# griffithlab/regtools

Measured on AMD Instinct MI355X. Metric: alignments/sec + junctions/sec, junctions extract, 1/2/4/8 MI355X, higher is better.
Workload: dtype u8/u32 integer; 1 GPU; configs[1]: synthetic 50000000-read 101 bp BAM per GPU, ~15% reads with one N-op, junctions extract -s XS; reads_per_gpu=50000000, seed=1, bgzf_members=169426, compressed_bytes_per_gpu=533101619, inflated_bytes_per_gpu=11060000978

## Files before the change

regtools_amd/csrc/api_internal.h:

```cpp
#pragma once
#include "../../include/regtools_amd.h"

#include <hip/hip_runtime.h>
#include <stdarg.h>
#include <stdio.h>
#include <stdlib.h>
#include <string.h>

#include <algorithm>
#include <atomic>
#include <condition_variable>
#include <charconv>
#include <chrono>
#include <map>
#include <memory>
#include <mutex>
#include <string>
#include <thread>
#include <unordered_map>
#include <vector>

#include "cse_host.h"
#include "host_io.h"
#include "worker_pool.h"
// ... 320 lines not shown
    CallIndex(const uint8_t *index, size_t index_len) : bai(index), bai_len(index_len), th([this] {
        ok = bai && normalize_index(bai, bai_len, image, bai, bai_len) && parse_bai(bai, bai_len, bi, false); }) {}
    void join() { if (th.joinable()) th.join(); }
    ~CallIndex() { join(); }
};

struct MemberDiscovery {
    rgx_ctx *c = nullptr; hipStream_t st = nullptr;
    const uint8_t *d_bam = nullptr; size_t bam_len = 0;
    const uint32_t *d_true_sizes = nullptr;
    Scalars *d_sc = nullptr, *h_sc = nullptr;
    uint32_t n_cand = 0;
    uint64_t *cand = nullptr;
    uint32_t *nx[2] = {nullptr, nullptr}, *c_isize = nullptr, *c_reach = nullptr, *c_rank = nullptr, *c_isz2 = nullptr, *c_tmp = nullptr;
    Member *d_members = nullptr;
    StageGuard g_cand, g_members;
    int candidates(bool guarded, char *err, size_t errlen) {
        DevBuf &b_disc = c->buf(Buf::discover), &b_cand = c->buf(Buf::cand), &b_members = c->buf(Buf::members);
        const uint32_t n_tiles = (uint32_t)((bam_len + kMagicTile - 1) / kMagicTile);
        HIP_TRY(b_disc.ensure((size_t)n_tiles * 4 + scan_tmp_words(n_tiles) * 4 + 256));
        Carve wd(b_disc);
        uint32_t *tile_cnt = wd.u32(n_tiles), *tile_tmp = wd.u32(scan_tmp_words(n_tiles)); CARVE_TRY(wd, "discover");
        launch_magic_count(d_bam, bam_len, n_tiles, tile_cnt, st);
        launch_scan_u32(tile_cnt, tile_cnt, n_tiles, &d_sc->n_cand, tile_tmp, st);
        HIP_TRY(fetch_scalar(d_sc, h_sc, h_sc->n_cand, st));
        HIP_TRY(hipStreamSynchronize(st));
        n_cand = h_sc->n_cand;
        if (n_cand == 0) return kGoOn;
        const size_t N = n_cand, guard_bytes = guarded ? kGuardWords * 4 : 0;
        HIP_TRY(b_cand.ensure(N * 8 + N * 4 * 6 + scan_tmp_words(n_cand) * 4 + guard_bytes + 256));
        HIP_TRY(b_members.ensure((N + 1) * sizeof(Member) + guard_bytes));
        Carve wc(b_cand);
        cand = wc.u64(n_cand);
        uint32_t *guard_at = guarded ? wc.u32(kGuardWords) : nullptr;
        nx[0] = wc.u32(n_cand); nx[1] = wc.u32(n_cand);
        c_isize = wc.u32(n_cand); c_reach = wc.u32(n_cand); c_rank = wc.u32(n_cand); c_isz2 = wc.u32(n_cand); c_tmp = wc.u32(scan_tmp_words(n_cand));
        CARVE_TRY(wc, "cand");
        d_members = b_members.as<Member>();
        if (guarded) { g_cand.arm(guard_at, st); g_members.arm((uint32_t *)(d_members + N), st); }
        launch_magic_fill(d_bam, bam_len, n_tiles, tile_cnt, cand, st);
        return kGoOn;
    }
    void chain(uint64_t root2) {
        launch_member_link(d_bam, bam_len, cand, n_cand, nx[0], c_isize, c_reach, root2, st);
        int cur = 0;
        for (uint32_t span = 1; span < n_cand; span <<= 1) { launch_member_jump(n_cand, nx[cur], nx[cur ^ 1], c_reach, st); cur ^= 1; }
        launch_member_jump(n_cand, nx[cur], nx[cur ^ 1], c_reach, st);
        launch_scan_u32(c_reach, c_rank, n_cand, &d_sc->n_members, c_tmp, st);
// ... 82 lines not shown
        if (!split_B) return hipSuccess;
        split_B = false;
        return hipStreamWaitEvent(st, split_ev, 0);
    }
    bool spec = false; uint32_t mean_rec = 0;
    BamHeader hdr; int32_t n_ref = 0;
    uint64_t lim = 0, pos0 = 0; bool chain_ended = false;
    ExtractCfg cfg{}; SegGeom geom{}; uint32_t seg_bytes = 0;
    std::vector<SegChunk> seg_chunks;
    const uint8_t *arena = nullptr; uint64_t span = 0; uint32_t n_seg = 0, n_rec = 0; bool lite_walk = false;
    uint64_t *seg_start[2] = {nullptr, nullptr}, *seg_exit[2] = {nullptr, nullptr};
    uint32_t *seg_cnt[2] = {nullptr, nullptr}, *seg_base = nullptr;
    uint32_t *seg_iter_e = nullptr, *seg_long_e = nullptr, *seg_long_base_e = nullptr;
    uint16_t *seg_cp = nullptr;
    int cur = 0;
    int frame(uint32_t n_s, uint32_t walk_from, bool &ended) {
        DevBuf &b_tmp = c->buf(Buf::tmp);
        launch_seg_walk(arena, geom, n_s, n_ref, seg_start[cur], seg_exit[cur], seg_cnt[cur], seg_cp, st, walk_from);
        for (int iter = 0;; ++iter) {
            HIP_TRY(hipMemsetAsync(&d_sc->framing, 0xff, sizeof d_sc->framing, st));
            launch_seg_verify(arena, geom, n_s, seg_start[cur], seg_exit[cur], seg_cnt[cur], seg_start[cur ^ 1], seg_exit[cur ^ 1],
                              seg_cnt[cur ^ 1], &d_sc->framing.disagree, seg_cp, st);
            cur ^= 1;
            launch_scan_u32(seg_cnt[cur], seg_base, n_s, &d_sc->n_rec, b_tmp.as<uint32_t>(), st);
            HIP_TRY(fetch(h_sc->n_rec));
            HIP_TRY(fetch(h_sc->framing));
            if (spec && iter == 0) HIP_TRY(fetch_verdict());
            HIP_TRY(hipStreamSynchronize(st));
            if (spec && iter == 0 && !verdict_clean()) {
                mark("inflate verdict: not clean, starting over device-resident");
                if (gated) { c->gate_distrust = true; if (trace) fprintf(stderr,
                    "[rgx trace] arrival gate: verdict not clean, this context no longer uses it\n"); }
                return restart(Restart::verdict_not_clean);
            }
            ++P.framing_sweeps;
            const Scalars::Framing &fr = h_sc->framing;
            if (fr.chain_end != 0xffffffffu) ended = true;
            if (fr.chain_end != 0xffffffffu && (fr.chain_end < fr.disagree || (fr.disagree == 0xffffffffu && geom.chunks))) {
                launch_seg_truncate(geom, n_s, fr.chain_end, seg_start[cur], seg_exit[cur], seg_cnt[cur], st);
                launch_scan_u32(seg_cnt[cur], seg_base, n_s, &d_sc->n_rec, b_tmp.as<uint32_t>(), st);
                HIP_TRY(fetch(h_sc->n_rec));
                HIP_TRY(hipStreamSynchronize(st));
                break;
            }
            if (fr.disagree == 0xffffffffu) break;
            if (iter > 1 << 20) return fail(err, errlen, RGX_ERR_FORMAT, "regtools_amd: record framing did not converge\n");
        }
        return kGoOn;
    }
    uint32_t sA = 0;
    bool emit_parts_ok = false; uint32_t emit_parts = 0, emit_rows = 0; size_t ev_lay = 0;
    EventSoA ev_e{};
    static constexpr size_t kEventRowBytes = 8 * sizeof(uint32_t) + 1;
    EventSoA ev_layout(Carve &w, size_t E) {
        EventSoA v; memset(&v, 0, sizeof v);
        v.tid = w.u32(E); v.start = w.u32(E); v.ilen_cls = w.u32(E); v.ts = w.u32(E); v.te = w.u32(E);
        if (want_read_span) { v.rpos = w.u32(E); v.rend = w.u32(E); }
        if (p->barcodes) v.read = w.u32(E);
        v.strand = w.u8(E);
        return v;
    }
    size_t soa_cap = 0;
    ReadSoA soa{};
    uint32_t *ev_base = nullptr, *long_list = nullptr;
// ... 58 lines not shown
```

regtools_amd/csrc/api_records.cpp:

```cpp
#include "api_internal.h"

int EventsRun::stage_footers_and_header() {
    DevBuf &b_arena = c->buf(Buf::arena), &b_hdr = c->buf(Buf::hdr_arena), &b_lens = c->buf(Buf::inflate_scratch);
    BamHeader hdr_host;
    spec = overlap && !d_true_sizes && !geom_chunked_hint && host_bam_header(h_bam, std::min<size_t>(bam_len, (size_t)8 << 20), hdr_host, nullptr, &mean_rec);
    if (spec) h_sc->inflate = h_sc->inflate_early = InflateStatus{0xffffffffu, 0xffffffffu};
    else {
        HIP_TRY(join_B());
        HIP_TRY(fetch_verdict());
        HIP_TRY(hipStreamSynchronize(st));
    }
    if (!d_true_sizes) {
        auto size_trouble = [](const InflateStatus &s) { return s.first_bad != 0xffffffffu &&
            (s.code == 12u  || s.code == 10u ); };
        bool lies = size_trouble(h_sc->inflate) || size_trouble(h_sc->inflate_early);
        if (!lies && stop < n_members_all) {
            Member ms; uint8_t two[2] = {0, 0};
            HIP_TRY(member_at(stop, ms));
            if (ms.isize == 0 && ms.clen >= 2) {
                if (h_bam && ms.cpos + 2 <= bam_len) memcpy(two, h_bam + ms.cpos, 2);
                else { HIP_TRY(hipMemcpyAsync(two, d_bam + ms.cpos, 2, hipMemcpyDeviceToHost, st)); HIP_TRY(hipStreamSynchronize(st)); }
            }
            lies = !(ms.isize == 0 && two[0] == 3 && two[1] == 0) && ms.isize != 0xffffffffu;
        }
// ... 234 lines not shown
            if (reaches_J && trace) fprintf(stderr,
                "[rgx trace] early tail: a record of the prefix ends at %llu, behind the inflated part (%llu): one pass\n", (unsigned long long)exit_J,
                (unsigned long long)ep.upos);
            const bool slow_J = P.framing_sweeps - sweeps0 > 2;
            P.framing_sweeps = sweeps0;
            const uint64_t span_J = (uint64_t)sJ * seg_bytes;
            if (h_sc->wait_timed_out) { c->early_distrust = true; if (trace) fprintf(stderr,
                "[rgx trace] early tail: a wait for a part's waves timed out, this context no longer uses it\n"); }
            if (h_sc->wait_timed_out || ended_J || slow_J || reaches_J || !n_rec_J || span_J / n_rec_J > kSparseRecordBytes ||
                (sA && n_rec_J > soa_cap)) { early = false; sA = 0; emit_parts_ok = false; emit_parts = 0; emit_rows = 0; break; }
            if (!sA) {
                { const int rc = soa_layout((size_t)((double)n_rec_J * ((double)n_seg / sJ) * 1.125) + 65536); if (rc != kGoOn) return rc; }
                if (lite_walk) { cfg.insane_out = &d_sc->insane; HIP_TRY(hipMemsetAsync(&d_sc->insane, 0, 4, st)); h_sc->insane = 0; }
            }
            launch_decode_seg(arena, geom, sJ, seg_start[cur], seg_base, seg_cnt[cur], cfg, soa, seg_iter_e, seg_long_e, seg_cp, true, st, sA);
            if (!sA) {
                DevBuf &b_ev0 = c->buf(Buf::events);
                ev_lay = b_ev0.cap > 256 ? (b_ev0.cap - 256) / kEventRowBytes : 0;
                emit_parts_ok = ev_lay >= 4096;
                if (emit_parts_ok) { HIP_TRY(b_tmp.ensure(scan_tmp_words((uint32_t)std::min<size_t>(soa_cap, 0xffffffffu)) * 4 + 64));
                    Carve w(b_ev0); ev_e = ev_layout(w, ev_lay); CARVE_TRY(w, "events"); }
            }
            if (emit_parts_ok && emit_parts < kGateParts - 1) {
                launch_scan_u32(soa.n_ev + emit_rows, ev_base + emit_rows, n_rec_J - emit_rows, d_sc->part_events + emit_parts, b_tmp.as<uint32_t>(), st);
                launch_emit_short(arena, n_rec_J, cfg, soa, ev_base, ev_e, st, emit_rows, d_sc->part_events, emit_parts, (uint32_t)std::min<size_t>(ev_lay,
                    0xffffffffu));
                emit_rows = n_rec_J; ++emit_parts;
            }
            sA = sJ;
            mark("early tail: part framed and decoded");
        }
        HIP_TRY(join_B());
        const int rcF = frame(n_seg, sA, chain_ended);
        if (rcF != kGoOn) return rcF;
        n_rec = h_sc->n_rec;
    } else HIP_TRY(join_B());
    if (spec && !n_seg) {
        HIP_TRY(fetch_verdict());
        HIP_TRY(hipStreamSynchronize(st));
        if (!verdict_clean()) {
            mark("inflate verdict: not clean, nothing framed, starting over device-resident");
            return restart(Restart::verdict_not_clean_unframed);
        }
    }
    if (chain_ended) P.stream_ended = true;
    if (chain_ended && geom.chunks && m_hi < n_members_all && !path.to_file_end) {
        mark("region: chain ended, re-reading to the end of the file");
// ... 4 lines not shown

    return kGoOn;
}

int EventsRun::stage_decode() {
    DevBuf &b_tmp = c->buf(Buf::tmp);
    if (n_rec) {
        const size_t R = n_rec;
        const uint32_t s_from = sA && (R > soa_cap || chain_ended) ? 0 : sA;
        if (!s_from) { const int rc = soa_layout(R); if (rc != kGoOn) return rc; emit_parts_ok = false; }
        HIP_TRY(b_tmp.ensure(scan_tmp_words(n_rec) * 4 + 64));
        uint32_t *seg_iter = sA ? seg_iter_e : seg_cnt[cur ^ 1], *seg_long = sA ? seg_long_e : (uint32_t *)seg_start[cur ^ 1], *seg_long_base = sA ?
            seg_long_base_e : (uint32_t *)seg_exit[cur ^ 1];
        if (geom.chunks) {
            cfg.stop_out = &d_sc->stop_rule.index; cfg.stop_index = 0xffffffffu;
            HIP_TRY(hipMemsetAsync(&d_sc->stop_rule.index, 0xff, 4, st));
            HIP_TRY(hipMemsetAsync(&d_sc->stop_rule.last_pass, 0, 4, st));
        }
        if (!s_from && lite_walk) { cfg.insane_out = &d_sc->insane; HIP_TRY(hipMemsetAsync(&d_sc->insane, 0, 4, st)); h_sc->insane = 0; }
        for (int pass = 0; pass < 2; ++pass) {
            launch_decode_seg(arena, geom, n_seg, seg_start[cur], seg_base, seg_cnt[cur], cfg, soa, seg_iter, seg_long, seg_cp,
                              span / n_rec <= kSparseRecordBytes, st, s_from);
            if (emit_parts_ok && s_from) {
                launch_scan_u32(soa.n_ev + emit_rows, ev_base + emit_rows, n_rec - emit_rows, d_sc->part_events + emit_parts, b_tmp.as<uint32_t>(), st);
                launch_emit_short(arena, n_rec, cfg, soa, ev_base, ev_e, st, emit_rows, d_sc->part_events, emit_parts,
                    (uint32_t)std::min<size_t>(ev_lay, 0xffffffffu));
                HIP_TRY(fetch(h_sc->part_events));
            } else launch_scan_u32(soa.n_ev, ev_base, n_rec, &d_sc->counts.n_events, b_tmp.as<uint32_t>(), st);
            launch_scan_u32(seg_iter, seg_iter, n_seg, &d_sc->counts.n_iterated, b_tmp.as<uint32_t>(), st);
            launch_scan_u32(seg_long, seg_long_base, n_seg, &d_sc->counts.n_long, b_tmp.as<uint32_t>(), st);
            HIP_TRY(fetch(h_sc->counts));
            if (cfg.stop_out) HIP_TRY(fetch(h_sc->stop_rule));
            if (cfg.insane_out) HIP_TRY(fetch(h_sc->insane));
            if (cfg.abort_out) HIP_TRY(fetch(h_sc->abort_row));
            if (cfg.odd_count) HIP_TRY(fetch(h_sc->odd_aux));
            HIP_TRY(hipStreamSynchronize(st));
            if (cfg.insane_out && h_sc->insane) {
                mark("decode: a record fails bam_read1's test, starting over with the full walk");
                return restart(Restart::record_fails_full_test);
            }
            if (pass || !cfg.stop_out || h_sc->stop_rule.index == 0xffffffffu || h_sc->stop_rule.last_pass <= h_sc->stop_rule.index + 1) break;
            cfg.stop_index = h_sc->stop_rule.index;
        }
        if (cfg.abort_out && h_sc->abort_row != 0xffffffffu && h_sc->abort_row < (cfg.stop_out ? cfg.stop_index : 0xffffffffu))
            return fail(err, errlen, RGX_ERR_ABORT,
                "regtools_amd: record %u has an auxiliary field of unknown type in front of its strand or barcode tag: the reference abort()s here\n",
                h_sc->abort_row);
        n_events = h_sc->counts.n_events; n_long = h_sc->counts.n_long;
        if (emit_parts_ok && s_from) {
            uint64_t tot = 0;
            for (uint32_t k = 0; k <= emit_parts && k < kGateParts; ++k) tot += h_sc->part_events[k];
            if (tot > ev_lay || tot > 0xffffffffull || n_long) {
                emit_parts_ok = false;
                launch_scan_u32(soa.n_ev, ev_base, n_rec, &d_sc->counts.n_events, b_tmp.as<uint32_t>(), st);
                HIP_TRY(fetch(h_sc->counts.n_events));
                HIP_TRY(hipStreamSynchronize(st));
                n_events = h_sc->counts.n_events;
            } else n_events = (uint32_t)tot;
        }
        n_iterated = h_sc->counts.n_iterated;
        if (cfg.odd_count && h_sc->odd_aux) {
            const uint32_t cap = h_sc->odd_aux;
            DevBuf &b_odd = c->buf(Buf::odd_aux);
            HIP_TRY(b_odd.ensure((size_t)cap * 12 + 16));
            HIP_TRY(hipMemsetAsync(&d_sc->odd_aux, 0, 4, st));
            launch_collect_odd_aux(arena, soa, n_rec, cap, &d_sc->odd_aux, b_odd.as<int32_t>(), st);
            HIP_TRY(fetch(h_sc->odd_aux));
            HIP_TRY(hipStreamSynchronize(st));
            const uint32_t n_odd = std::min(h_sc->odd_aux, cap);
            std::vector<int32_t> rows((size_t)n_odd * 3);
            if (n_odd) { HIP_TRY(hipMemcpyAsync(rows.data(), b_odd.p, (size_t)n_odd * 12, hipMemcpyDeviceToHost, st)); HIP_TRY(hipStreamSynchronize(st)); }
            for (uint32_t k = 0; k < n_odd; ++k) P.odd_aux.push_back(Prep::OddAux{rows[3 * (size_t)k], rows[3 * (size_t)k + 1], rows[3 * (size_t)k + 2]});
        }
        if (geom.chunks && p->n_shards > 1 && h_sc->stop_rule.index != 0xffffffffu) P.stream_ended = true;
        if (n_long) launch_long_fill(n_seg, seg_base, seg_cnt[cur], seg_long_base, cfg, soa, long_list, st);
    }
    HIP_TRY(hipEventRecord(c->ev[4], st));
    mark("decode+count (sync)");
// ... 49 lines not shown
```

regtools_amd/csrc/api_reduce.cpp:

```cpp
#include "api_internal.h"

int reduce_events(rgx_ctx *c, EventSoA ev, uint32_t n_events, uint32_t group_bits, uint32_t ilen_bits, const uint32_t *rank_of_group_host,
                         uint32_t n_groups, HostRows &R, char *err, size_t errlen, bool view_only, RowMap *row_map, TableSink *sink, bool allow_preagg) {
    hipStream_t st = c->stream;
    Scalars *d_sc = c->buf(Buf::scalars).as<Scalars>(), *h_sc = (Scalars *)c->pinned;
    DevBuf &b_sort = c->buf(Buf::sort), &b_uni = c->buf(Buf::unique);
    c->last_rows_valid = false;
    uint32_t n_unique = 0;
    UniqueSoA u; memset(&u, 0, sizeof u);
    const uint32_t *final_perm = nullptr;
    uint32_t *chrom_rank_rows = nullptr;
    R = HostRows();
    if (n_events) {
        const bool preagg = !row_map && allow_preagg;
        PartialSoA pr; memset(&pr, 0, sizeof pr);
        uint32_t *ev_flag = nullptr, *ev_flag_tmp = nullptr;
        EventSoA sev = ev;
        uint32_t n_s = n_events;
        if (preagg) {
            DevBuf &b_par = c->buf(Buf::partials);
            const size_t Ev = n_events;
            HIP_TRY(b_par.ensure(Ev * 4 * 9 + scan_tmp_words(n_events) * 4 + 512));
            Carve q(b_par);
            pr.tid = q.u32(Ev); pr.start = q.u32(Ev); pr.ilen_cls = q.u32(Ev); pr.ts = q.u32(Ev); pr.te = q.u32(Ev);
            pr.count = q.u32(Ev); pr.first = q.u32(Ev); pr.last = q.u32(Ev); ev_flag = q.u32(Ev); ev_flag_tmp = q.u32(scan_tmp_words(n_events));
            CARVE_TRY(q, "partials");
            HIP_TRY(hipMemsetAsync(&d_sc->counts.n_partial, 0, 4, st));
            launch_preagg(ev, n_events, pr, &d_sc->counts.n_partial, st);
            HIP_TRY(fetch_scalar(d_sc, h_sc, h_sc->counts.n_partial, st));
            HIP_TRY(hipStreamSynchronize(st));
            n_s = h_sc->counts.n_partial;
            memset(&sev, 0, sizeof sev);
            sev.tid = pr.tid; sev.start = pr.start; sev.ilen_cls = pr.ilen_cls; sev.ts = pr.ts; sev.te = pr.te;
        }
        const size_t E = n_s;
        const size_t rtmp = radix_tmp_words(n_s) + scan_tmp_words(n_s) + 64;
        HIP_TRY(b_sort.ensure(E * 4 * 6 + rtmp * 4 + 256));
        Carve q(b_sort);
        uint32_t *perm0 = q.u32(E), *perm1 = q.u32(E), *key0 = q.u32(E), *key1 = q.u32(E);
        uint32_t *head = q.u32(E), *seg_excl = q.u32(E), *tmp = q.u32(rtmp); CARVE_TRY(q, "sort");
        RadixSort by_key{{perm0, perm1}, tmp, n_s, st, {key0, key1}};
        by_key.by_keyed(sev.ilen_cls, ilen_bits);
        by_key.by_keyed(sev.start, 32);
        by_key.by_keyed(sev.tid, group_bits);
        const uint32_t *sorted = by_key.sorted();
        launch_heads(sev, sorted, n_s, head, st);
        launch_scan_u32(head, seg_excl, n_s, &d_sc->counts.n_unique, tmp, st);
        HIP_TRY(fetch_scalar(d_sc, h_sc, h_sc->counts.n_unique, st));
        HIP_TRY(hipStreamSynchronize(st));
        n_unique = h_sc->counts.n_unique;

        const size_t U = n_unique;
        const size_t utmp = radix_tmp_words(n_unique) + 64;
        HIP_TRY(b_uni.ensure(U * 4 * 13 + U + utmp * 4 + 256));
        Carve w(b_uni);
        u.tid = w.u32(U); u.start = w.u32(U); u.end = w.u32(U); u.ts_min = w.u32(U); u.te_max = w.u32(U); u.count = w.u32(U);
        u.first_seen = w.u32(U); u.last_seen = w.u32(U); u.name_rank = w.u32(U);
        uint32_t *head_pos = w.u32(U); chrom_rank_rows = w.u32(U);
        uint32_t *uperm0 = w.u32(U), *uperm1 = w.u32(U), *utmp_p = w.u32(utmp);
        u.strand = w.u8(U); CARVE_TRY(w, "unique");
        launch_fill_u32(u.ts_min, 0xffffffffu, U, st);
        launch_fill_u32(u.te_max, 0u, U, st);
        if (preagg) {
            launch_fill_u32(u.count, 0u, U, st);
            launch_fill_u32(u.first_seen, 0xffffffffu, U, st);
            launch_fill_u32(u.last_seen, 0u, U, st);
            launch_reduce_partials(pr, sorted, head, seg_excl, n_s, u, st);
            HIP_TRY(hipMemsetAsync(ev_flag, 0, (size_t)n_events * 4, st));
            launch_reduce_finish_partials(ev.strand, n_unique, u, ev_flag, st);
            launch_scan_u32(ev_flag, ev_flag, n_events, nullptr, ev_flag_tmp, st);
            launch_name_rank(n_unique, ev_flag, u, st);
        } else {
            launch_reduce(ev, sorted, head, seg_excl, n_events, u, head_pos, st);
            if (row_map) {
                DevBuf &b_map = c->buf(Buf::row_map);
                HIP_TRY(b_map.ensure((E + U) * 4 + 256));
                Carve wm(b_map);
                row_map->ev_urow = wm.u32(E); row_map->urow_pos = wm.u32(U); CARVE_TRY(wm, "row_map");
                launch_event_urow(sorted, head, seg_excl, n_events, row_map->ev_urow, st);
            }
            uint32_t *first_flag = head;
            HIP_TRY(hipMemsetAsync(first_flag, 0, E * 4, st));
            launch_reduce_finish(ev, sorted, n_events, n_unique, head_pos, u, first_flag, st);
            launch_scan_u32(first_flag, seg_excl, n_events, nullptr, tmp, st);
            launch_name_rank(n_unique, seg_excl, u, st);
        }

        uint32_t rk = 0;
        for (uint32_t i = 0; i < n_groups; ++i) rk = std::max(rk, rank_of_group_host[i]);
// ... 71 lines not shown
    b.len = q.u32(E); b.h_lo = q.u32(E); b.h_hi = q.u32(E); b.row = q.u32(E);
    uint32_t *perm0 = q.u32(E), *perm1 = q.u32(E), *head = q.u32(E), *seg_excl = q.u32(E);
    uint32_t *pair_row = q.u32(E), *pair_first = q.u32(E), *pair_pos = q.u32(E), *pair_len = q.u32(E), *pair_count = q.u32(E);
    uint32_t *tmp = q.u32(rtmp); CARVE_TRY(q, "barcodes");
    uint32_t *flags = &d_sc->barcodes.not_string;
    HIP_TRY(hipMemsetAsync(flags, 0, 8, st));
    launch_bc_event_keys(P.arena, (uint32_t)E, P.ev.read, P.soa.rec_off, rm.ev_urow, rm.urow_pos, (uint8_t)p->barcode_tag[0], (uint8_t)p->barcode_tag[1], b,
        flags, st);
    RadixSort by_key{{perm0, perm1}, tmp, (uint32_t)E, st};
    by_key.by(b.h_lo, 32); by_key.by(b.h_hi, 32);
    by_key.by(b.row, std::max<uint32_t>(1, bitlen((uint32_t)std::max<size_t>(U, 1) - 1)));
    const uint32_t *sorted = by_key.sorted();
    launch_bc_heads(P.arena, b, sorted, (uint32_t)E, head, flags, st);
    launch_scan_u32(head, seg_excl, (uint32_t)E, &d_sc->barcodes.n_pairs, tmp, st);
    HIP_TRY(fetch_scalar(d_sc, h_sc, h_sc->barcodes, st));
    HIP_TRY(hipStreamSynchronize(st));
    if (h_sc->barcodes.not_string) return fail(err, errlen, RGX_ERR_FORMAT,
        "regtools_amd: the %c%c tag of an alignment is not a string (the reference dies on such input)\n\n", p->barcode_tag[0], p->barcode_tag[1]);
    if (h_sc->barcodes.hash_clash) return fail(err, errlen, RGX_ERR_DEVICE, "regtools_amd: two different barcodes of one junction share a 64-bit hash; not handled\n\n");
    const uint32_t n_pairs = h_sc->barcodes.n_pairs;
    launch_bc_pairs(b, sorted, head, seg_excl, (uint32_t)E, pair_row, pair_first, pair_pos, pair_off, pair_len, st);
    launch_bc_counts(n_pairs, (uint32_t)E, pair_pos, pair_count, st);
    uint32_t *str_begin = head;
    launch_scan_u32(pair_len, str_begin, n_pairs, &d_sc->barcode_text_len, tmp, st);
    HIP_TRY(fetch_scalar(d_sc, h_sc, h_sc->barcode_text_len, st));
    HIP_TRY(hipStreamSynchronize(st));
    const size_t text_len = h_sc->barcode_text_len;
    DevBuf &b_txt = c->buf(Buf::barcode_text);
    HIP_TRY(b_txt.ensure(text_len + 256));
    launch_bc_gather(P.arena, n_pairs, pair_off, pair_len, str_begin, b_txt.as<uint8_t>(), st);
    std::vector<uint32_t> h_row(n_pairs), h_first(n_pairs), h_count(n_pairs), h_begin(n_pairs), h_len(n_pairs);
    std::vector<char> h_text(text_len + 1);
    HIP_TRY(hipMemcpyAsync(h_row.data(), pair_row, (size_t)n_pairs * 4, hipMemcpyDeviceToHost, st));
    HIP_TRY(hipMemcpyAsync(h_first.data(), pair_first, (size_t)n_pairs * 4, hipMemcpyDeviceToHost, st));
    HIP_TRY(hipMemcpyAsync(h_count.data(), pair_count, (size_t)n_pairs * 4, hipMemcpyDeviceToHost, st));
    HIP_TRY(hipMemcpyAsync(h_begin.data(), str_begin, (size_t)n_pairs * 4, hipMemcpyDeviceToHost, st));
    HIP_TRY(hipMemcpyAsync(h_len.data(), pair_len, (size_t)n_pairs * 4, hipMemcpyDeviceToHost, st));
    if (text_len) HIP_TRY(hipMemcpyAsync(h_text.data(), b_txt.p, text_len, hipMemcpyDeviceToHost, st));
    HIP_TRY(hipStreamSynchronize(st));

    t->bc_count = (uint32_t *)calloc((size_t)n_pairs + 1, 4);
    t->bc_str_begin = (uint64_t *)calloc((size_t)n_pairs + 1, 8);
    t->bc_text = (char *)malloc(text_len + 1);
    t->bc_insert_rank = (uint32_t *)calloc((size_t)n_pairs + 1, 4);
    std::vector<uint32_t> rank_of(n_pairs);
    std::vector<uint32_t> run_begin(U + 1, 0);
    for (uint32_t k = 0; k < n_pairs; ++k) run_begin[h_row[k] + 1]++;
    for (size_t r = 0; r < U; ++r) run_begin[r + 1] += run_begin[r];
// ... 101 lines not shown
```

regtools_amd/csrc/kernels.h:

```cpp
#pragma once
#include <hip/hip_runtime.h>

#include "common.h"
#include "bam_core.h"
#include "front_plan.h"

namespace rgx {

constexpr uint32_t kSegBytes = 16384;
constexpr uint32_t kSparseRecordBytes = 2048;
constexpr uint32_t kSegCpSlots = 64;
constexpr uint64_t kChainEnd = ~0ull;
constexpr uint64_t kChainUnknown = ~0ull - 1;

size_t inflate_scratch_bytes(uint32_t n_members);
hipError_t pending_launch_error();
struct InflateGate {
    const uint32_t *flags = nullptr;
    uint32_t epoch = 0;
    uint32_t n_chunks = 0;
    uint64_t lo = 0, chunk_bytes = 1;
    uint32_t *done = nullptr;
    uint32_t part_start[7] = {0xffffffffu, 0xffffffffu, 0xffffffffu, 0xffffffffu, 0xffffffffu, 0xffffffffu, 0xffffffffu};
};
// ... 65 lines not shown

void launch_decode_seg(const uint8_t *arena, SegGeom g, uint32_t n_seg, const uint64_t *seg_start, const uint32_t *seg_base,
                       const uint32_t *seg_cnt, ExtractCfg cfg, ReadSoA soa, uint32_t *seg_iter, uint32_t *seg_long, const uint16_t *seg_cp,
                       bool staged , hipStream_t stream,
                       uint32_t s_begin = 0 );
void launch_long_fill(uint32_t n_seg, const uint32_t *seg_base, const uint32_t *seg_cnt, const uint32_t *seg_long_base, ExtractCfg cfg, ReadSoA soa,
                      uint32_t *long_list, hipStream_t stream);

struct EventSoA {
    uint32_t *tid, *start, *ilen_cls;
    uint32_t *ts, *te;
    uint32_t *rpos, *rend;
    uint8_t  *strand;
    uint32_t *read;
};
void launch_emit_short(const uint8_t *arena, uint32_t n_rec, ExtractCfg cfg, ReadSoA soa, const uint32_t *ev_base,
                       EventSoA ev, hipStream_t stream, uint32_t row_begin = 0 ,
                       const uint32_t *part_totals = nullptr, uint32_t n_parts = 0 ,
                       uint32_t slot_cap = 0xffffffffu );
void launch_emit_long(const uint8_t *arena, const uint32_t *long_list, uint32_t n_long,
                      ExtractCfg cfg, ReadSoA soa, const uint32_t *ev_base, EventSoA ev, hipStream_t stream);

size_t scan_tmp_words(uint32_t n);
void launch_scan_u32(const uint32_t *in, uint32_t *out, uint32_t n, uint32_t *total, uint32_t *tmp, hipStream_t stream);

size_t radix_tmp_words(uint32_t n);
void launch_radix_pass(const uint32_t *word, uint32_t shift, uint32_t bits, const uint32_t *perm_in, uint32_t *perm_out,
                       uint32_t n, uint32_t *tmp, hipStream_t stream);
void launch_radix_pass_keyed(const uint32_t *key_in, uint32_t *key_out, uint32_t shift, uint32_t bits, const uint32_t *perm_in, uint32_t *perm_out,
                             uint32_t n, uint32_t *tmp, hipStream_t stream);

struct UniqueSoA {
    uint32_t *tid, *start, *end, *ts_min, *te_max, *count, *first_seen, *last_seen, *name_rank;
    uint8_t  *strand;
};
struct PartialSoA { uint32_t *tid, *start, *ilen_cls, *ts, *te, *count, *first, *last; };
void launch_preagg(EventSoA ev, uint32_t n, PartialSoA p, uint32_t *p_total , hipStream_t stream);
void launch_reduce_partials(PartialSoA p, const uint32_t *perm, const uint32_t *head, const uint32_t *seg_excl, uint32_t n, UniqueSoA u, hipStream_t stream);
void launch_reduce_finish_partials(const uint8_t *ev_strand, uint32_t n_unique, UniqueSoA u, uint32_t *first_flag , hipStream_t stream);
void launch_heads(EventSoA ev, const uint32_t *perm, uint32_t n, uint32_t *head, hipStream_t stream);
void launch_reduce(EventSoA ev, const uint32_t *perm, const uint32_t *head, const uint32_t *seg_excl, uint32_t n, UniqueSoA u,
                   uint32_t *head_pos, hipStream_t stream);
void launch_reduce_finish(EventSoA ev, const uint32_t *perm, uint32_t n, uint32_t n_unique, const uint32_t *head_pos, UniqueSoA u,
                          uint32_t *first_flag, hipStream_t stream);
void launch_name_rank(uint32_t n_unique, const uint32_t *flag_scan, UniqueSoA u, hipStream_t stream);
void launch_gather_u32(uint32_t n, const uint32_t *table, const uint32_t *idx, uint32_t *out, hipStream_t stream);
void launch_fill_u32(uint32_t *p, uint32_t v, size_t n, hipStream_t stream);
void launch_rows_out(UniqueSoA u, const uint32_t *order, uint32_t n, uint32_t *out, hipStream_t stream);
RGX_HD size_t table_block_rows(uint64_t n) { return ((size_t)n + 1 + 15) & ~(size_t)15; }
RGX_HD size_t table_block_bytes(uint64_t n) { return table_block_rows(n) * (8 * 3 + 4 * 6 + 3); }
void launch_rows_table(UniqueSoA u, const uint32_t *order, uint32_t n, uint32_t min_anchor, uint8_t *out, hipStream_t stream);


struct BarcodeEv { uint64_t *off; uint32_t *len, *h_lo, *h_hi, *row; };
void launch_event_urow(const uint32_t *sorted, const uint32_t *head, const uint32_t *seg_excl, uint32_t n, uint32_t *ev_urow, hipStream_t stream);
void launch_inverse_perm(const uint32_t *perm, uint32_t n, uint32_t *inv, hipStream_t stream);
void launch_bc_event_keys(const uint8_t *arena, uint32_t n_events, const uint32_t *ev_read, const uint64_t *rec_off, const uint32_t *ev_urow,
                          const uint32_t *urow_pos, uint8_t t0, uint8_t t1, BarcodeEv b, uint32_t *flags, hipStream_t stream);
void launch_bc_heads(const uint8_t *arena, BarcodeEv b, const uint32_t *perm, uint32_t n, uint32_t *head, uint32_t *flags, hipStream_t stream);
void launch_bc_pairs(BarcodeEv b, const uint32_t *perm, const uint32_t *head, const uint32_t *seg_excl, uint32_t n, uint32_t *pair_row,
// ... 149 lines not shown
```

regtools_amd/csrc/prims_kernels.hip:

```cpp
#include "wave_prims.h"

#include <algorithm>

namespace rgx {

constexpr uint32_t kScanTile = 4096;

__global__ __launch_bounds__(256) void k_scan_reduce(const uint32_t *__restrict__ in, uint32_t n, uint32_t *tile_sum) {
    __shared__ uint32_t s_wave[4];
    const uint32_t base = blockIdx.x * kScanTile + threadIdx.x * 16;
    uint32_t sum = 0;
#pragma unroll
    for (uint32_t k = 0; k < 16; ++k) sum += (base + k < n) ? in[base + k] : 0u;
    uint32_t tot; block_excl_scan_256(sum, s_wave, tot);
    if (threadIdx.x == 0) tile_sum[blockIdx.x] = tot;
}

__global__ __launch_bounds__(256) void k_scan_tiles(uint32_t *tile_sum, uint32_t n_tiles, uint32_t *total) {
    __shared__ uint32_t s_wave[4];
    uint32_t carry = 0;
    for (uint32_t base = 0; base < n_tiles; base += 256) {
        const uint32_t i = base + threadIdx.x;
        const uint32_t v = i < n_tiles ? tile_sum[i] : 0u;
        uint32_t tot; const uint32_t ex = block_excl_scan_256(v, s_wave, tot);
        if (i < n_tiles) tile_sum[i] = carry + ex;
        carry += tot;
    }
    if (threadIdx.x == 0 && total) *total = carry;
}

__global__ __launch_bounds__(256) void k_scan_apply(const uint32_t *__restrict__ in, uint32_t *out, uint32_t n, const uint32_t *__restrict__ tile_sum) {
    __shared__ uint32_t s_wave[4];
    const uint32_t base = blockIdx.x * kScanTile + threadIdx.x * 16;
    uint32_t v[16], sum = 0;
#pragma unroll
    for (uint32_t k = 0; k < 16; ++k) { v[k] = (base + k < n) ? in[base + k] : 0u; sum += v[k]; }
    uint32_t tot; uint32_t run = block_excl_scan_256(sum, s_wave, tot) + tile_sum[blockIdx.x];
#pragma unroll
    for (uint32_t k = 0; k < 16; ++k) { if (base + k < n) out[base + k] = run; run += v[k]; }
}

size_t scan_tmp_words(uint32_t n) { return (size_t)(n + kScanTile - 1) / kScanTile + 1; }

void launch_scan_u32(const uint32_t *in, uint32_t *out, uint32_t n, uint32_t *total, uint32_t *tmp, hipStream_t stream) {
    if (!n) { if (total) (void)hipMemsetAsync(total, 0, 4, stream); return; }
    const uint32_t tiles = (n + kScanTile - 1) / kScanTile;
    hipLaunchKernelGGL(k_scan_reduce, dim3(tiles), dim3(256), 0, stream, in, n, tmp);
    hipLaunchKernelGGL(k_scan_tiles, dim3(1), dim3(256), 0, stream, tmp, tiles, total);
    hipLaunchKernelGGL(k_scan_apply, dim3(tiles), dim3(256), 0, stream, in, out, n, tmp);
}

constexpr uint32_t kRadixRowsLarge = 32, kRadixRowsSmall = 8, kRadixSmallMax = 2u << 20;
static inline uint32_t radix_rows(uint32_t n) {
    return n <= kRadixSmallMax ? kRadixRowsSmall : kRadixRowsLarge;
}

__device__ __forceinline__ uint32_t radix_digit(const uint32_t *__restrict__ word, const uint32_t *__restrict__ perm_in, uint32_t i,
                                                uint32_t shift, uint32_t mask, uint32_t &src) {
    src = perm_in ? perm_in[i] : i;
    return (word[src] >> shift) & mask;
}

__device__ __forceinline__ uint64_t match_digit(uint32_t d, bool valid) {
    uint64_t m = __ballot(valid);
#pragma unroll
    for (uint32_t b = 0; b < 8; ++b) {
        const uint64_t bal = __ballot((d >> b) & 1u);
        m &= ((d >> b) & 1u) ? bal : ~bal;
    }
    return m;
}
// ... 102 lines not shown
```

regtools_amd/csrc/reduce_kernels.hip:

```cpp
#include "wave_prims.h"

namespace rgx {

__global__ void k_heads(EventSoA ev, const uint32_t *__restrict__ perm, uint32_t n, uint32_t *head) {
    const uint32_t i = blockIdx.x * blockDim.x + threadIdx.x;
    if (i >= n) return;
    uint32_t h = 1;
    if (i > 0) {
        const uint32_t a = perm[i], b = perm[i - 1];
        h = (ev.tid[a] != ev.tid[b]) || (ev.start[a] != ev.start[b]) || (ev.ilen_cls[a] != ev.ilen_cls[b]);
    }
    head[i] = h;
}

__global__ void k_reduce(EventSoA ev, const uint32_t *__restrict__ perm, const uint32_t *__restrict__ head,
                         const uint32_t *__restrict__ seg_excl, uint32_t n, UniqueSoA u, uint32_t *head_pos) {
    const uint32_t i = blockIdx.x * blockDim.x + threadIdx.x;
    const bool valid = i < n;
    uint32_t row = 0, ts = 0xffffffffu, te = 0, hd = 0;
    if (valid) {
        const uint32_t e = perm[i];
        hd = head[i];
        row = seg_excl[i] + hd - 1;
        ts = ev.ts[e]; te = ev.te[e];
// ... 137 lines not shown
__device__ __forceinline__ void table_row(uint8_t *out, size_t m, uint32_t i, uint32_t tid, uint32_t start, uint32_t end, uint32_t ts, uint32_t te, uint32_t count,
                                          uint64_t name_index, uint64_t first, uint64_t last, uint32_t strand, uint32_t min_anchor) {
    uint64_t *q8 = (uint64_t *)out;
    q8[i] = name_index; q8[m + i] = first; q8[2 * m + i] = last;
    uint32_t *q4 = (uint32_t *)(out + m * 24);
    q4[i] = tid; q4[m + i] = start; q4[2 * m + i] = end; q4[3 * m + i] = ts; q4[4 * m + i] = te; q4[5 * m + i] = count;
    uint8_t *q1 = out + m * 48;
    q1[i] = (uint8_t)strand;
    q1[m + i] = (uint32_t)(start - ts) >= min_anchor;
    q1[2 * m + i] = (uint32_t)(te - end) >= min_anchor;
}
__global__ void k_rows_table(UniqueSoA u, const uint32_t *__restrict__ order, uint32_t n, uint32_t min_anchor, uint8_t *out) {
    const uint32_t i = blockIdx.x * blockDim.x + threadIdx.x;
    if (i >= n) return;
    const uint32_t s = order[i];
    table_row(out, table_block_rows(n), i, u.tid[s], u.start[s], u.end[s], u.ts_min[s], u.te_max[s], u.count[s], u.name_rank[s], u.first_seen[s], u.last_seen[s], u.strand[s], min_anchor);
}

__global__ void k_fill_u32(uint32_t *p, uint32_t v, size_t n) {
    const size_t i = (size_t)blockIdx.x * blockDim.x + threadIdx.x;
    if (i < n) p[i] = v;
}

void launch_heads(EventSoA ev, const uint32_t *perm, uint32_t n, uint32_t *head, hipStream_t stream) {
    if (n) hipLaunchKernelGGL(k_heads, dim3((n + 255) / 256), dim3(256), 0, stream, ev, perm, n, head);
}
void launch_reduce(EventSoA ev, const uint32_t *perm, const uint32_t *head, const uint32_t *seg_excl, uint32_t n, UniqueSoA u,
                   uint32_t *head_pos, hipStream_t stream) {
    if (n) hipLaunchKernelGGL(k_reduce, dim3((n + 255) / 256), dim3(256), 0, stream, ev, perm, head, seg_excl, n, u, head_pos);
}
void launch_reduce_finish(EventSoA ev, const uint32_t *perm, uint32_t n, uint32_t n_unique, const uint32_t *head_pos, UniqueSoA u,
                          uint32_t *first_flag, hipStream_t stream) {
    if (n_unique) hipLaunchKernelGGL(k_reduce_finish, dim3((n_unique + 255) / 256), dim3(256), 0, stream, ev, perm, n, n_unique, head_pos, u, first_flag);
}
void launch_name_rank(uint32_t n_unique, const uint32_t *flag_scan, UniqueSoA u, hipStream_t stream) {
    if (n_unique) hipLaunchKernelGGL(k_name_rank, dim3((n_unique + 255) / 256), dim3(256), 0, stream, n_unique, flag_scan, u);
}
void launch_gather_u32(uint32_t n, const uint32_t *table, const uint32_t *idx, uint32_t *out, hipStream_t stream) {
    if (n) hipLaunchKernelGGL(k_gather_u32, dim3((n + 255) / 256), dim3(256), 0, stream, n, table, idx, out);
}
void launch_rows_out(UniqueSoA u, const uint32_t *order, uint32_t n, uint32_t *out, hipStream_t stream) {
    if (n) hipLaunchKernelGGL(k_rows_out, dim3((n + 255) / 256), dim3(256), 0, stream, u, order, n, out);
}
void launch_rows_table(UniqueSoA u, const uint32_t *order, uint32_t n, uint32_t min_anchor, uint8_t *out, hipStream_t stream) {
    if (n) hipLaunchKernelGGL(k_rows_table, dim3((n + 255) / 256), dim3(256), 0, stream, u, order, n, min_anchor, out);
}
// ... 16 lines not shown
```

Before: 2.187 billion alignments/s.

## Fuse scan tile pass into reduce via last-block counter and write totals to host

```diff
diff --git a/regtools_amd/csrc/api_internal.h b/regtools_amd/csrc/api_internal.h
--- a/regtools_amd/csrc/api_internal.h
+++ b/regtools_amd/csrc/api_internal.h
@@ -366,8 +366,7 @@
         Carve wd(b_disc);
         uint32_t *tile_cnt = wd.u32(n_tiles), *tile_tmp = wd.u32(scan_tmp_words(n_tiles)); CARVE_TRY(wd, "discover");
         launch_magic_count(d_bam, bam_len, n_tiles, tile_cnt, st);
-        launch_scan_u32(tile_cnt, tile_cnt, n_tiles, &d_sc->n_cand, tile_tmp, st);
-        HIP_TRY(fetch_scalar(d_sc, h_sc, h_sc->n_cand, st));
+        launch_scan_u32(tile_cnt, tile_cnt, n_tiles, &d_sc->n_cand, tile_tmp, st, &h_sc->n_cand);
         HIP_TRY(hipStreamSynchronize(st));
         n_cand = h_sc->n_cand;
         if (n_cand == 0) return kGoOn;
@@ -496,8 +495,7 @@
             launch_seg_verify(arena, geom, n_s, seg_start[cur], seg_exit[cur], seg_cnt[cur], seg_start[cur ^ 1], seg_exit[cur ^ 1],
                               seg_cnt[cur ^ 1], &d_sc->framing.disagree, seg_cp, st);
             cur ^= 1;
-            launch_scan_u32(seg_cnt[cur], seg_base, n_s, &d_sc->n_rec, b_tmp.as<uint32_t>(), st);
-            HIP_TRY(fetch(h_sc->n_rec));
+            launch_scan_u32(seg_cnt[cur], seg_base, n_s, &d_sc->n_rec, b_tmp.as<uint32_t>(), st, &h_sc->n_rec);
             HIP_TRY(fetch(h_sc->framing));
             if (spec && iter == 0) HIP_TRY(fetch_verdict());
             HIP_TRY(hipStreamSynchronize(st));
@@ -512,8 +510,7 @@
             if (fr.chain_end != 0xffffffffu) ended = true;
             if (fr.chain_end != 0xffffffffu && (fr.chain_end < fr.disagree || (fr.disagree == 0xffffffffu && geom.chunks))) {
                 launch_seg_truncate(geom, n_s, fr.chain_end, seg_start[cur], seg_exit[cur], seg_cnt[cur], st);
-                launch_scan_u32(seg_cnt[cur], seg_base, n_s, &d_sc->n_rec, b_tmp.as<uint32_t>(), st);
-                HIP_TRY(fetch(h_sc->n_rec));
+                launch_scan_u32(seg_cnt[cur], seg_base, n_s, &d_sc->n_rec, b_tmp.as<uint32_t>(), st, &h_sc->n_rec);
                 HIP_TRY(hipStreamSynchronize(st));
                 break;
             }
diff --git a/regtools_amd/csrc/api_records.cpp b/regtools_amd/csrc/api_records.cpp
--- a/regtools_amd/csrc/api_records.cpp
+++ b/regtools_amd/csrc/api_records.cpp
@@ -280,7 +280,8 @@
                     Carve w(b_ev0); ev_e = ev_layout(w, ev_lay); CARVE_TRY(w, "events"); }
             }
             if (emit_parts_ok && emit_parts < kGateParts - 1) {
-                launch_scan_u32(soa.n_ev + emit_rows, ev_base + emit_rows, n_rec_J - emit_rows, d_sc->part_events + emit_parts, b_tmp.as<uint32_t>(), st);
+                launch_scan_u32(soa.n_ev + emit_rows, ev_base + emit_rows, n_rec_J - emit_rows, d_sc->part_events + emit_parts, b_tmp.as<uint32_t>(), st,
+                                h_sc->part_events + emit_parts);
                 launch_emit_short(arena, n_rec_J, cfg, soa, ev_base, ev_e, st, emit_rows, d_sc->part_events, emit_parts, (uint32_t)std::min<size_t>(ev_lay,
                     0xffffffffu));
                 emit_rows = n_rec_J; ++emit_parts;
@@ -331,14 +332,13 @@
             launch_decode_seg(arena, geom, n_seg, seg_start[cur], seg_base, seg_cnt[cur], cfg, soa, seg_iter, seg_long, seg_cp,
                               span / n_rec <= kSparseRecordBytes, st, s_from);
             if (emit_parts_ok && s_from) {
-                launch_scan_u32(soa.n_ev + emit_rows, ev_base + emit_rows, n_rec - emit_rows, d_sc->part_events + emit_parts, b_tmp.as<uint32_t>(), st);
+                launch_scan_u32(soa.n_ev + emit_rows, ev_base + emit_rows, n_rec - emit_rows, d_sc->part_events + emit_parts, b_tmp.as<uint32_t>(), st,
+                                h_sc->part_events + emit_parts);
                 launch_emit_short(arena, n_rec, cfg, soa, ev_base, ev_e, st, emit_rows, d_sc->part_events, emit_parts,
                     (uint32_t)std::min<size_t>(ev_lay, 0xffffffffu));
-                HIP_TRY(fetch(h_sc->part_events));
-            } else launch_scan_u32(soa.n_ev, ev_base, n_rec, &d_sc->counts.n_events, b_tmp.as<uint32_t>(), st);
-            launch_scan_u32(seg_iter, seg_iter, n_seg, &d_sc->counts.n_iterated, b_tmp.as<uint32_t>(), st);
-            launch_scan_u32(seg_long, seg_long_base, n_seg, &d_sc->counts.n_long, b_tmp.as<uint32_t>(), st);
-            HIP_TRY(fetch(h_sc->counts));
+            } else launch_scan_u32(soa.n_ev, ev_base, n_rec, &d_sc->counts.n_events, b_tmp.as<uint32_t>(), st, &h_sc->counts.n_events);
+            launch_scan_u32(seg_iter, seg_iter, n_seg, &d_sc->counts.n_iterated, b_tmp.as<uint32_t>(), st, &h_sc->counts.n_iterated);
+            launch_scan_u32(seg_long, seg_long_base, n_seg, &d_sc->counts.n_long, b_tmp.as<uint32_t>(), st, &h_sc->counts.n_long);
             if (cfg.stop_out) HIP_TRY(fetch(h_sc->stop_rule));
             if (cfg.insane_out) HIP_TRY(fetch(h_sc->insane));
             if (cfg.abort_out) HIP_TRY(fetch(h_sc->abort_row));
@@ -361,8 +361,7 @@
             for (uint32_t k = 0; k <= emit_parts && k < kGateParts; ++k) tot += h_sc->part_events[k];
             if (tot > ev_lay || tot > 0xffffffffull || n_long) {
                 emit_parts_ok = false;
-                launch_scan_u32(soa.n_ev, ev_base, n_rec, &d_sc->counts.n_events, b_tmp.as<uint32_t>(), st);
-                HIP_TRY(fetch(h_sc->counts.n_events));
+                launch_scan_u32(soa.n_ev, ev_base, n_rec, &d_sc->counts.n_events, b_tmp.as<uint32_t>(), st, &h_sc->counts.n_events);
                 HIP_TRY(hipStreamSynchronize(st));
                 n_events = h_sc->counts.n_events;
             } else n_events = (uint32_t)tot;
diff --git a/regtools_amd/csrc/api_reduce.cpp b/regtools_amd/csrc/api_reduce.cpp
--- a/regtools_amd/csrc/api_reduce.cpp
+++ b/regtools_amd/csrc/api_reduce.cpp
@@ -45,8 +45,7 @@
         by_key.by_keyed(sev.tid, group_bits);
         const uint32_t *sorted = by_key.sorted();
         launch_heads(sev, sorted, n_s, head, st);
-        launch_scan_u32(head, seg_excl, n_s, &d_sc->counts.n_unique, tmp, st);
-        HIP_TRY(fetch_scalar(d_sc, h_sc, h_sc->counts.n_unique, st));
+        launch_scan_u32(head, seg_excl, n_s, &d_sc->counts.n_unique, tmp, st, &h_sc->counts.n_unique);
         HIP_TRY(hipStreamSynchronize(st));
         n_unique = h_sc->counts.n_unique;
 
@@ -59,12 +58,8 @@
         uint32_t *head_pos = w.u32(U); chrom_rank_rows = w.u32(U);
         uint32_t *uperm0 = w.u32(U), *uperm1 = w.u32(U), *utmp_p = w.u32(utmp);
         u.strand = w.u8(U); CARVE_TRY(w, "unique");
-        launch_fill_u32(u.ts_min, 0xffffffffu, U, st);
-        launch_fill_u32(u.te_max, 0u, U, st);
+        launch_fill_unique(u, n_unique, preagg, st);
         if (preagg) {
-            launch_fill_u32(u.count, 0u, U, st);
-            launch_fill_u32(u.first_seen, 0xffffffffu, U, st);
-            launch_fill_u32(u.last_seen, 0u, U, st);
             launch_reduce_partials(pr, sorted, head, seg_excl, n_s, u, st);
             HIP_TRY(hipMemsetAsync(ev_flag, 0, (size_t)n_events * 4, st));
             launch_reduce_finish_partials(ev.strand, n_unique, u, ev_flag, st);
@@ -182,8 +177,7 @@
     launch_bc_pairs(b, sorted, head, seg_excl, (uint32_t)E, pair_row, pair_first, pair_pos, pair_off, pair_len, st);
     launch_bc_counts(n_pairs, (uint32_t)E, pair_pos, pair_count, st);
     uint32_t *str_begin = head;
-    launch_scan_u32(pair_len, str_begin, n_pairs, &d_sc->barcode_text_len, tmp, st);
-    HIP_TRY(fetch_scalar(d_sc, h_sc, h_sc->barcode_text_len, st));
+    launch_scan_u32(pair_len, str_begin, n_pairs, &d_sc->barcode_text_len, tmp, st, &h_sc->barcode_text_len);
     HIP_TRY(hipStreamSynchronize(st));
     const size_t text_len = h_sc->barcode_text_len;
     DevBuf &b_txt = c->buf(Buf::barcode_text);
diff --git a/regtools_amd/csrc/kernels.h b/regtools_amd/csrc/kernels.h
--- a/regtools_amd/csrc/kernels.h
+++ b/regtools_amd/csrc/kernels.h
@@ -111,7 +111,7 @@
                       ExtractCfg cfg, ReadSoA soa, const uint32_t *ev_base, EventSoA ev, hipStream_t stream);
 
 size_t scan_tmp_words(uint32_t n);
-void launch_scan_u32(const uint32_t *in, uint32_t *out, uint32_t n, uint32_t *total, uint32_t *tmp, hipStream_t stream);
+void launch_scan_u32(const uint32_t *in, uint32_t *out, uint32_t n, uint32_t *total, uint32_t *tmp, hipStream_t stream, uint32_t *total_host = nullptr);
 
 size_t radix_tmp_words(uint32_t n);
 void launch_radix_pass(const uint32_t *word, uint32_t shift, uint32_t bits, const uint32_t *perm_in, uint32_t *perm_out,
@@ -125,6 +125,7 @@
 };
 struct PartialSoA { uint32_t *tid, *start, *ilen_cls, *ts, *te, *count, *first, *last; };
 void launch_preagg(EventSoA ev, uint32_t n, PartialSoA p, uint32_t *p_total , hipStream_t stream);
+void launch_fill_unique(UniqueSoA u, uint32_t n, bool partials, hipStream_t stream);
 void launch_reduce_partials(PartialSoA p, const uint32_t *perm, const uint32_t *head, const uint32_t *seg_excl, uint32_t n, UniqueSoA u, hipStream_t stream);
 void launch_reduce_finish_partials(const uint8_t *ev_strand, uint32_t n_unique, UniqueSoA u, uint32_t *first_flag , hipStream_t stream);
 void launch_heads(EventSoA ev, const uint32_t *perm, uint32_t n, uint32_t *head, hipStream_t stream);
diff --git a/regtools_amd/csrc/prims_kernels.hip b/regtools_amd/csrc/prims_kernels.hip
--- a/regtools_amd/csrc/prims_kernels.hip
+++ b/regtools_amd/csrc/prims_kernels.hip
@@ -1,52 +1,115 @@
 #include "wave_prims.h"
 
 #include <algorithm>
+#include <map>
+#include <mutex>
+#include <utility>
 
 namespace rgx {
 
 constexpr uint32_t kScanTile = 4096;
 
-__global__ __launch_bounds__(256) void k_scan_reduce(const uint32_t *__restrict__ in, uint32_t n, uint32_t *tile_sum) {
-    __shared__ uint32_t s_wave[4];
-    const uint32_t base = blockIdx.x * kScanTile + threadIdx.x * 16;
+typedef uint32_t ScanVec __attribute__((ext_vector_type(4), aligned(4)));
+
+__device__ __forceinline__ uint4 scan_load4(const uint32_t *in, uint32_t i, uint32_t n) {
+    if (i < n && n - i >= 4) { const ScanVec v = *(const ScanVec *)(in + i); return make_uint4(v.x, v.y, v.z, v.w); }
+    return make_uint4(i < n ? in[i] : 0u, i < n && n - i > 1 ? in[i + 1] : 0u, i < n && n - i > 2 ? in[i + 2] : 0u, 0u);
+}
+__device__ __forceinline__ void scan_store4(uint32_t *out, uint32_t i, uint32_t n, uint4 v) {
+    if (i < n && n - i >= 4) { ScanVec w; w.x = v.x; w.y = v.y; w.z = v.z; w.w = v.w; *(ScanVec *)(out + i) = w; return; }
+    if (i < n) out[i] = v.x;
+    if (i < n && n - i > 1) out[i + 1] = v.y;
+    if (i < n && n - i > 2) out[i + 2] = v.z;
+}
+
+__global__ __launch_bounds__(256) void k_scan_reduce(const uint32_t *__restrict__ in, uint32_t n, uint32_t *tile_sum, uint32_t n_tiles, uint32_t *total,
+                                                     uint32_t *total_host, uint32_t *counter) {
+    __shared__ uint32_t s_wave[4], s_last;
+    if (!n) { if (threadIdx.x == 0) { if (total) *total = 0; if (total_host) *total_host = 0; } return; }
+    const uint32_t tile0 = blockIdx.x * kScanTile;
     uint32_t sum = 0;
 #pragma unroll
-    for (uint32_t k = 0; k < 16; ++k) sum += (base + k < n) ? in[base + k] : 0u;
+    for (uint32_t r = 0; r < 4; ++r) { const uint4 v = scan_load4(in, tile0 + (r * 256 + threadIdx.x) * 4, n); sum += v.x + v.y + v.z + v.w; }
     uint32_t tot; block_excl_scan_256(sum, s_wave, tot);
-    if (threadIdx.x == 0) tile_sum[blockIdx.x] = tot;
-}
-
-__global__ __launch_bounds__(256) void k_scan_tiles(uint32_t *tile_sum, uint32_t n_tiles, uint32_t *total) {
-    __shared__ uint32_t s_wave[4];
+    if (threadIdx.x == 0) {
+        __hip_atomic_store(&tile_sum[blockIdx.x], tot, __ATOMIC_RELAXED, __HIP_MEMORY_SCOPE_AGENT);
+        asm volatile("s_waitcnt vmcnt(0)" ::: "memory");
+        s_last = __hip_atomic_fetch_add(counter, 1u, __ATOMIC_RELAXED, __HIP_MEMORY_SCOPE_AGENT) == n_tiles - 1;
+    }
+    __syncthreads();
+    if (!s_last) return;
     uint32_t carry = 0;
     for (uint32_t base = 0; base < n_tiles; base += 256) {
         const uint32_t i = base + threadIdx.x;
-        const uint32_t v = i < n_tiles ? tile_sum[i] : 0u;
-        uint32_t tot; const uint32_t ex = block_excl_scan_256(v, s_wave, tot);
+        const uint32_t v = i < n_tiles ? __hip_atomic_load(&tile_sum[i], __ATOMIC_RELAXED, __HIP_MEMORY_SCOPE_AGENT) : 0u;
+        uint32_t t2; const uint32_t ex = block_excl_scan_256(v, s_wave, t2);
         if (i < n_tiles) tile_sum[i] = carry + ex;
-        carry += tot;
-    }
-    if (threadIdx.x == 0 && total) *total = carry;
-}
-
-__global__ __launch_bounds__(256) void k_scan_apply(const uint32_t *__restrict__ in, uint32_t *out, uint32_t n, const uint32_t *__restrict__ tile_sum) {
+        carry += t2;
+    }
+    if (threadIdx.x == 0) {
+        if (total) *total = carry;
+        if (total_host) *total_host = carry;
+        __hip_atomic_store(counter, 0u, __ATOMIC_RELAXED, __HIP_MEMORY_SCOPE_AGENT);
+    }
+}
+
+constexpr uint32_t kScanLdsWords = kScanTile / 16 * 20;
+__device__ __forceinline__ uint32_t scan_lds_at(uint32_t chunk ) { return 4 * (chunk + (chunk >> 2)); }
+
+__global__ __launch_bounds__(256) void k_scan_apply(const uint32_t *in, uint32_t *out, uint32_t n, const uint32_t *__restrict__ tile_sum) {
     __shared__ uint32_t s_wave[4];
-    const uint32_t base = blockIdx.x * kScanTile + threadIdx.x * 16;
-    uint32_t v[16], sum = 0;
-#pragma unroll
-    for (uint32_t k = 0; k < 16; ++k) { v[k] = (base + k < n) ? in[base + k] : 0u; sum += v[k]; }
+    __shared__ __attribute__((aligned(16))) uint32_t s_x[kScanLdsWords];
+    const uint32_t tile0 = blockIdx.x * kScanTile, t = threadIdx.x;
+#pragma unroll
+    for (uint32_t r = 0; r < 4; ++r) { const uint32_t c = r * 256 + t; *(uint4 *)&s_x[scan_lds_at(c)] = scan_load4(in, tile0 + c * 4, n); }
+    __syncthreads();
+    uint4 v[4]; uint32_t sum = 0;
+#pragma unroll
+    for (uint32_t k = 0; k < 4; ++k) { v[k] = *(const uint4 *)&s_x[20 * t + 4 * k]; sum += v[k].x + v[k].y + v[k].z + v[k].w; }
     uint32_t tot; uint32_t run = block_excl_scan_256(sum, s_wave, tot) + tile_sum[blockIdx.x];
 #pragma unroll
-    for (uint32_t k = 0; k < 16; ++k) { if (base + k < n) out[base + k] = run; run += v[k]; }
+    for (uint32_t k = 0; k < 4; ++k) {
+        uint4 e; e.x = run; run += v[k].x; e.y = run; run += v[k].y; e.z = run; run += v[k].z; e.w = run; run += v[k].w;
+        *(uint4 *)&s_x[20 * t + 4 * k] = e;
+    }
+    __syncthreads();
+#pragma unroll
+    for (uint32_t r = 0; r < 4; ++r) { const uint32_t c = r * 256 + t; scan_store4(out, tile0 + c * 4, n, *(const uint4 *)&s_x[scan_lds_at(c)]); }
 }
 
 size_t scan_tmp_words(uint32_t n) { return (size_t)(n + kScanTile - 1) / kScanTile + 1; }
 
-void launch_scan_u32(const uint32_t *in, uint32_t *out, uint32_t n, uint32_t *total, uint32_t *tmp, hipStream_t stream) {
-    if (!n) { if (total) (void)hipMemsetAsync(total, 0, 4, stream); return; }
+constexpr size_t kCounterSlab = 1024;
+static uint32_t *stream_counter(hipStream_t stream) {
+    struct Slab { uint32_t *words = nullptr; size_t used = kCounterSlab; };
+    static std::mutex mu;
+    static std::map<std::pair<int, hipStream_t>, uint32_t *> word_of;
+    static std::map<int, Slab> slab_of;
+    int dev = 0;
+    if (hipGetDevice(&dev) != hipSuccess) return nullptr;
+    std::lock_guard<std::mutex> lock(mu);
+    uint32_t *&w = word_of[std::make_pair(dev, stream)];
+    if (w) return w;
+    Slab &s = slab_of[dev];
+    if (s.used == kCounterSlab) {
+        static const uint32_t zeros[kCounterSlab] = {};
+        void *p = nullptr;
+        if (hipMalloc(&p, sizeof zeros) != hipSuccess) return nullptr;
+        if (hipMemcpy(p, zeros, sizeof zeros, hipMemcpyHostToDevice) != hipSuccess) { (void)hipFree(p); return nullptr; }
+        s.words = (uint32_t *)p; s.used = 0;
+    }
+    return w = s.words + s.used++;
+}
+
+void launch_scan_u32(const uint32_t *in, uint32_t *out, uint32_t n, uint32_t *total, uint32_t *tmp, hipStream_t stream, uint32_t *total_host) {
+    if (!n) {
+        if (total || total_host) hipLaunchKernelGGL(k_scan_reduce, dim3(1), dim3(256), 0, stream, in, 0u, tmp, 0u, total, total_host, (uint32_t *)nullptr);
+        return;
+    }
+    uint32_t *counter = stream_counter(stream);
+    if (!counter) return;
     const uint32_t tiles = (n + kScanTile - 1) / kScanTile;
-    hipLaunchKernelGGL(k_scan_reduce, dim3(tiles), dim3(256), 0, stream, in, n, tmp);
-    hipLaunchKernelGGL(k_scan_tiles, dim3(1), dim3(256), 0, stream, tmp, tiles, total);
+    hipLaunchKernelGGL(k_scan_reduce, dim3(tiles), dim3(256), 0, stream, in, n, tmp, tiles, total, total_host, counter);
     hipLaunchKernelGGL(k_scan_apply, dim3(tiles), dim3(256), 0, stream, in, out, n, tmp);
 }
 
diff --git a/regtools_amd/csrc/reduce_kernels.hip b/regtools_amd/csrc/reduce_kernels.hip
--- a/regtools_amd/csrc/reduce_kernels.hip
+++ b/regtools_amd/csrc/reduce_kernels.hip
@@ -183,6 +183,16 @@
     if (i < n) p[i] = v;
 }
 
+__global__ void k_fill_unique(UniqueSoA u, uint32_t n, bool partials) {
+    const uint32_t i = blockIdx.x * blockDim.x + threadIdx.x;
+    if (i >= n) return;
+    u.ts_min[i] = 0xffffffffu; u.te_max[i] = 0u;
+    if (partials) { u.count[i] = 0u; u.first_seen[i] = 0xffffffffu; u.last_seen[i] = 0u; }
+}
+
+void launch_fill_unique(UniqueSoA u, uint32_t n, bool partials, hipStream_t stream) {
+    if (n) hipLaunchKernelGGL(k_fill_unique, dim3((n + 255) / 256), dim3(256), 0, stream, u, n, partials);
+}
 void launch_heads(EventSoA ev, const uint32_t *perm, uint32_t n, uint32_t *head, hipStream_t stream) {
     if (n) hipLaunchKernelGGL(k_heads, dim3((n + 255) / 256), dim3(256), 0, stream, ev, perm, n, head);
 }
```

New measurement: 2.175 billion alignments/s, median of 2. No clear change (-0.6%).
